# OpenVVC/OpenVVC

Measured on AMD Instinct MI355X. Metric: decoded frames/sec, full rcn back-end decode step (H2D of the recorded picture + MC incl. BDOF/DMVR/affine-PROF/GPM/CIIP + LMCS + inverse transform + ordered intra pass + deblocking + SAO + ALF/CC-ALF + D2H of refined MVs + wait + per-picture digest + publication to the device DPB), 4K 10-bit RA rec, higher is better.
Workload: dtype u16 samples / int16 coefficients / int32 accumulate

## Files before the change

openvvc_amd/csrc/kernels_mc.hip:

```cpp
#include "mc_common.hip.h"
#include <stdlib.h>

#ifndef OV_WPE_MC
#define OV_WPE_MC 8
#endif
#if OV_WPE_MC > 0
#define OV_OCC_MC __attribute__((amdgpu_waves_per_eu(OV_WPE_MC)))
#else
#define OV_OCC_MC
#endif

namespace {

__device__ __forceinline__ int mc_gpm(uint32_t aux, int x, int y, int p0, int p1)
{
    const int k = (int16_t)(aux & 0xffff), a = (int8_t)((aux >> 16) & 0xff), b = (int8_t)(aux >> 24);
    const int wgt = ov_clip3((k + __mul24(a, x) + __mul24(b, y)) >> 3, 0, 8);
    return ov_clip_bd((__mul24(p1, 8 - wgt) + __mul24(p0, wgt) + 64) >> 7);
}

struct Combine { int a0, a1, rnd, sh; };
__device__ __forceinline__ Combine mc_combine_of(const ovhip_mc_unit &u)
{
    Combine c;
    if (u.dir != 3)                 { c.a0 = u.dir == 1; c.a1 = u.dir != 1; c.rnd = 8; c.sh = 4; }
    else if (u.w0 == 4 && u.w1 == 4) { c.a0 = 1; c.a1 = 1; c.rnd = 16; c.sh = 5; }
    else                            { c.a0 = u.w0; c.a1 = u.w1; c.rnd = 64; c.sh = 7; }
    return c;
}
__device__ __forceinline__ int mc_combine(const Combine &c, int p0, int p1) { return ov_clip_bd((__mul24(p1, c.a1) + __mul24(p0, c.a0) + c.rnd) >> c.sh); }

__device__ __forceinline__ int ciip_blend(int inter, int intra, int wt) { return ov_clip_bd((__mul24(intra, wt) + __mul24(inter, 4 - wt) + 2) >> 2); }

#define HLS 26
template <int NOUT>
__device__ __forceinline__ void luma_finish(const ovhip_mc_unit &u, const ovhip_pic &dst, const int16_t *s_hl, const int tv[2][4],
                                            int lane, int log2w, const uint16_t *__restrict__ lmcs_fwd, const ovhip_pic &intra)
{
    const int w = 1 << log2w;
    const int x = lane & (w - 1), yg = lane >> log2w, y0 = yg * NOUT;
    if (y0 >= u.h) return;
    int P[2][NOUT];
#pragma unroll
    for (int l = 0; l < 2; ++l) {
#pragma unroll
        for (int o = 0; o < NOUT; ++o) P[l][o] = 0;
        if (u.dir & (1 << l)) v_outputs<8, NOUT>(s_hl + l * 16 * HLS + x * HLS, y0, tv[l], P[l]);
    }
    uint16_t *d = dst.y + ov_rowoff(u.y + y0, dst.stride_y) + u.x + x;
    int v[NOUT];
    if (u.flags & OVHIP_MC_GPM) {
#pragma unroll
        for (int j = 0; j < NOUT; ++j) v[j] = mc_gpm(u.aux, x, y0 + j, P[0][j], P[1][j]);
    } else {
        const Combine cmb = mc_combine_of(u);
#pragma unroll
        for (int j = 0; j < NOUT; ++j) v[j] = mc_combine(cmb, P[0][j], P[1][j]);
    }
    if ((u.flags & OVHIP_MC_LMCS) && lmcs_fwd) {
#pragma unroll
        for (int j = 0; j < NOUT; ++j) v[j] = lmcs_fwd[v[j]];
    }
    if (!(u.flags & OVHIP_MC_GPM) && u.aux) {
        const uint16_t *ip = intra.y + ov_rowoff(u.y + y0, intra.stride_y) + u.x + x;
#pragma unroll
        for (int j = 0; j < NOUT; ++j) v[j] = ciip_blend(v[j], ip[j * intra.stride_y], u.aux & 7);
    }
#pragma unroll
    for (int j = 0; j < NOUT; ++j) d[j * dst.stride_y] = (uint16_t)v[j];
}

template <int NOUT>
__device__ __forceinline__ void chroma_finish(const ovhip_mc_unit &u, const ovhip_pic &dst, const int16_t *s_hc, const int tv[2][2],
                                              int lane, int log2wc, int hc, const ovhip_pic &intra)
{
    const int wc = 1 << log2wc;
    const int per_plane = (wc * hc) / NOUT;
    const int plane = lane >= per_plane, ll = lane - plane * per_plane;
    if (lane >= 2 * per_plane) return;
    const int x = ll & (wc - 1), y0 = (ll >> log2wc) * NOUT;
    int P[2][NOUT];
#pragma unroll
    for (int l = 0; l < 2; ++l) {
#pragma unroll
        for (int o = 0; o < NOUT; ++o) P[l][o] = 0;
        if (u.dir & (1 << l)) v_outputs<4, NOUT>(s_hc + (plane * 2 + l) * 8 * CHT_STRIDE + x * CHT_STRIDE, y0, tv[l], P[l]);
    }
    uint16_t *d = (plane ? dst.cr : dst.cb) + ov_rowoff((u.y >> 1) + y0, dst.stride_c) + (u.x >> 1) + x;
    const bool ciip = !(u.flags & OVHIP_MC_GPM) && u.aux && !(u.aux & 0x100);
    const uint16_t *ip = ciip ? (plane ? intra.cr : intra.cb) + ov_rowoff((u.y >> 1) + y0, intra.stride_c) + (u.x >> 1) + x : nullptr;
    int v[NOUT];
    if (u.flags & OVHIP_MC_GPM) {
#pragma unroll
        for (int j = 0; j < NOUT; ++j) v[j] = mc_gpm(u.aux, 2 * x, 2 * (y0 + j), P[0][j], P[1][j]);
    } else {
        const Combine cmb = mc_combine_of(u);
#pragma unroll
        for (int j = 0; j < NOUT; ++j) v[j] = mc_combine(cmb, P[0][j], P[1][j]);
    }
    if (ciip) {
#pragma unroll
        for (int j = 0; j < NOUT; ++j) v[j] = ciip_blend(v[j], ip[j * intra.stride_c], u.aux & 7);
    }
#pragma unroll
    for (int j = 0; j < NOUT; ++j) d[j * dst.stride_c] = (uint16_t)v[j];
}

#ifdef OV_MC_PHASES
#define OV_MC_PHASE_UNITS 65536
__device__ unsigned int g_mc_phase[OV_MC_PHASE_UNITS * 8];
#define OV_PHASE(i) do { __builtin_amdgcn_s_waitcnt(0); const unsigned long long t_ = __builtin_readcyclecounter(); \
                         ph[i] = t_ - tprev; tprev = t_; } while (0)
#else
#define OV_PHASE(i) do { } while (0)
#endif

__global__ __launch_bounds__(64) OV_OCC_MC void k_mc2(ovhip_pic dst, RefTable refs, const ovhip_mc_unit *__restrict__ units,
                                             uint32_t n_units, const uint16_t *__restrict__ lmcs_fwd, int xcd, ovhip_pic intra)
{
    constexpr int HL_STRIDE = HLS;
    constexpr int R2 = 2 * 16 * HL_STRIDE > 4 * CHR_WIN ? 2 * 16 * HL_STRIDE : 4 * CHR_WIN;
    __shared__ __attribute__((aligned(16))) uint16_t s_all[2 * LUMA_WIN + R2 + 4 * 8 * CHT_STRIDE + 8];
    uint16_t *const s_wl = s_all;
    uint16_t *const s_wc = s_all + 2 * LUMA_WIN;
    int16_t  *const s_hl = reinterpret_cast<int16_t *>(s_all + 2 * LUMA_WIN);
    int16_t  *const s_hc = reinterpret_cast<int16_t *>(s_all + 2 * LUMA_WIN + R2);
    static_assert(sizeof(s_all) <= 5120, "k_mc2 LDS block must stay under the 32-workgroups-per-CU step");

    const int lane = threadIdx.x;
    {
    const uint32_t wg = blockIdx.x;
    if (wg >= n_units) return;
    const uint32_t bid = xcd ? ov_xcd_slot(wg, n_units) : wg;
#ifdef OV_MC_PHASES
    unsigned long long ph[8] = {}, tprev = __builtin_readcyclecounter();
#endif
    const ovhip_mc_unit u = units[bid];
    OV_PHASE(0);

    const bool do_l = !(u.flags & OVHIP_MC_NO_LUMA), do_c = !(u.flags & OVHIP_MC_NO_CHROMA);
    const int w = u.w, h = u.h, wc = w >> 1, hc = h >> 1;
    const int log2w = 31 - __clz(w), log2wc = log2w - 1;
    const int nl = u.dir == 3 ? 2 : 1, l0 = u.dir == 2 ? 1 : 0;

    const int ri0 = (u.dir & 1) ? u.ref0 : u.ref1, ri1 = (u.dir & 2) ? u.ref1 : u.ref0;
    const uint16_t *const ry[2]  = { refs.p[ri0].y,  refs.p[ri1].y };
    const uint16_t *const rcb[2] = { refs.p[ri0].cb, refs.p[ri1].cb };
    const uint16_t *const rcr[2] = { refs.p[ri0].cr, refs.p[ri1].cr };
    int lx[2], ly[2], cx[2], cy[2];
#pragma unroll
    for (int l = 0; l < 2; ++l) {
        const int mvx = l ? u.mv1x : u.mv0x, mvy = l ? u.mv1y : u.mv0y;
        lx[l] = u.x + (mvx >> 4) - 3;        ly[l] = u.y + (mvy >> 4) - 3;
        cx[l] = (u.x >> 1) + (mvx >> 5) - 1; cy[l] = (u.y >> 1) + (mvy >> 5) - 1;
    }
    const uint32_t (*const ltab)[4] = (u.flags & OVHIP_MC_FILT_4x4) ? g_taps.luma4 : g_taps.luma;
    const bool hpel = !(u.flags & OVHIP_MC_FILT_4x4) && (u.flags & OVHIP_MC_HPEL_FILT);
    const int hl_l = l0 + (nl == 2 ? lane >> 5 : 0);
    const int hc_q = lane >> (nl == 2 ? 4 : 5);
    const int hc_l = l0 + (nl == 2 ? (hc_q & 1) : 0);
    int fxl = (hl_l ? u.mv1x : u.mv0x) & 15;
    if (hpel && fxl == 8) fxl = 16;
    const int fxc = (hc_l ? u.mv1x : u.mv0x) & 31;
    const uint4 hl_tp = *reinterpret_cast<const uint4 *>(ltab[fxl]);
    const uint2 hc_tp = *reinterpret_cast<const uint2 *>(g_taps.chroma[fxc]);
    uint16_t *const lwin[2] = { s_wl, s_wl + LUMA_WIN };
    uint16_t *const cwin[4] = { s_wc, s_wc + CHR_WIN, s_wc + 2 * CHR_WIN, s_wc + 3 * CHR_WIN };
    int offl[2], offc1[2];
    stage_unit_windows(dst, ry, rcb, rcr, lx, ly, cx, cy, w, h, u.dir, do_l, do_c, lane, lwin, WIN_STRIDE, cwin, CWIN_STRIDE, offl, offc1);
    const int offc[2][2] = { { offc1[0], offc1[1] }, { offc1[0], offc1[1] } };
    __syncthreads();
    OV_PHASE(2);

    if (do_c) {
        const int log2seg = log2wc > 2 ? log2wc - 2 : 0;
        const int l2per = nl == 2 ? 4 : 5;
        const int qi = hc_q, tl = lane & ((1 << l2per) - 1);
        const int plane = nl == 2 ? qi >> 1 : qi, l = hc_l;
        const int tp[2] = { (int)hc_tp.x, (int)hc_tp.y };
        const int off = plane ? (l ? offc[1][1] : offc[1][0]) : (l ? offc[0][1] : offc[0][0]);
        const bool ident = fxc == 0;
        const uint16_t *src = s_wc + (plane * 2 + l) * CHR_WIN;
        int16_t *ht = s_hc + (plane * 2 + l) * 8 * CHT_STRIDE;
        const int x0 = (tl & ((1 << log2seg) - 1)) << 2, rstep = (1 << l2per) >> log2seg;
        for (int r = tl >> log2seg; r < hc + 3; r += rstep) h_task<4>(src + r * CWIN_STRIDE, off, x0, tp, ident, ht, CHT_STRIDE, r);
    }
    __syncthreads();
    if (do_l) {
        const int log2seg = log2w > 2 ? log2w - 2 : 0;
        const int l2per = nl == 2 ? 5 : 6;
        const int tl = lane & ((1 << l2per) - 1), l = hl_l;
        const int tp[4] = { (int)hl_tp.x, (int)hl_tp.y, (int)hl_tp.z, (int)hl_tp.w };
        const int off = l ? offl[1] : offl[0];
        const bool ident = fxl == 0;
        const uint16_t *src = s_wl + l * LUMA_WIN;
        int16_t *ht = s_hl + l * 16 * HL_STRIDE;
        const int x0 = (tl & ((1 << log2seg) - 1)) << 2, rstep = (1 << l2per) >> log2seg;
        for (int r = tl >> log2seg; r < h + 7; r += rstep) h_task<8>(src + r * WIN_STRIDE, off, x0, tp, ident, ht, HL_STRIDE, r);
    }
    __syncthreads();
    OV_PHASE(3);

    int tvl[2][4], tvc[2][2];
#pragma unroll
    for (int l = 0; l < 2; ++l) {
        const int mvy = l ? u.mv1y : u.mv0y;
        int fy = mvy & 15;
        if (hpel && fy == 8) fy = 16;
        load_taps<4>(ltab[fy], tvl[l]);
        load_taps<2>(g_taps.chroma[mvy & 31], tvc[l]);
    }
    if (do_l) {
        const int npix = w * h;
        if (npix >= 256)      luma_finish<4>(u, dst, s_hl, tvl, lane, log2w, lmcs_fwd, intra);
        else if (npix >= 128) luma_finish<2>(u, dst, s_hl, tvl, lane, log2w, lmcs_fwd, intra);
        else                  luma_finish<1>(u, dst, s_hl, tvl, lane, log2w, lmcs_fwd, intra);
    }
    if (do_c) {
        if (wc * hc >= 64) chroma_finish<2>(u, dst, s_hc, tvc, lane, log2wc, hc, intra);
        else               chroma_finish<1>(u, dst, s_hc, tvc, lane, log2wc, hc, intra);
    }
    __syncthreads();
#ifdef OV_MC_PHASES
    { const unsigned long long t_ = __builtin_readcyclecounter(); ph[4] = t_ - tprev; tprev = t_; }
    OV_PHASE(5);
    if (lane == 0 && bid < OV_MC_PHASE_UNITS) {
#pragma unroll
        for (int i = 0; i < 6; ++i) g_mc_phase[bid * 8 + i] = (unsigned int)ph[i];
        g_mc_phase[bid * 8 + 7] = 1;
    }
#endif
    }
}

__global__ __launch_bounds__(256) void k_ciip(ovhip_pic dst, ovhip_pic intra, const ovhip_ciip_unit *__restrict__ units, uint32_t n)
{
    for (uint32_t bid = blockIdx.x; bid < n; bid += gridDim.x) {
        const ovhip_ciip_unit u = units[bid];
#pragma unroll
        for (int plane = 0; plane < 3; ++plane) {
            const int c = plane != 0;
            if (c && u.chroma_inter) continue;
            const int lw = u.log2_w - c, w = 1 << lw, npix = w << (u.log2_h - c);
            int ds, is;
            uint16_t *d = ov_plane(dst, plane, ds) + (u.y >> c) * ds + (u.x >> c);
            const uint16_t *s = ov_plane(intra, plane, is) + (u.y >> c) * is + (u.x >> c);
            for (int t = threadIdx.x; t < npix; t += 256) {
                const int x = t & (w - 1), y = t >> lw;
                d[y * ds + x] = (uint16_t)ov_clip_bd((s[y * is + x] * u.wt + d[y * ds + x] * (4 - u.wt) + 2) >> 2);
            }
        }
    }
}

}

#ifdef OV_MC_PHASES
extern "C" int ovhip_debug_mc_phases(unsigned int *out )
{
    return hipMemcpyFromSymbol(out, HIP_SYMBOL(g_mc_phase), sizeof(unsigned int) * OV_MC_PHASE_UNITS * 8) == hipSuccess ? OVHIP_OK : OVHIP_ELAUNCH;
}
#endif

extern "C" int ovhip_ciip_launch(ovhip_ctx *ctx, const ovhip_pic *dst, const ovhip_pic *intra,
                                 const ovhip_ciip_unit *d_units, uint32_t n_units)
{
    if (!ctx || !dst || !intra) return OVHIP_EINVAL;
    OV_DEVICE(ctx);
    if (!n_units) return OVHIP_OK;
    if (!d_units) return ov_fail(ctx, OVHIP_EINVAL, "ovhip_ciip_launch: null units", hipSuccess);
    hipLaunchKernelGGL(k_ciip, dim3(n_units), dim3(256), 0, ctx->stream, *dst, *intra, d_units, n_units);
    OV_LAUNCH_CHECK(ctx, "k_ciip");
    return OVHIP_OK;
}

extern "C" int ovhip_mc_launch(ovhip_ctx *ctx, const ovhip_pic *dst, const ovhip_pic *refs, uint32_t n_refs,
                               const ovhip_mc_unit *d_units, uint32_t n_units, const uint16_t *d_lmcs_fwd_lut,
                               const ovhip_pic *intra)
{
    if (!ctx || !dst) return OVHIP_EINVAL;
    OV_DEVICE(ctx);
    if (!n_units) return OVHIP_OK;
    if (!refs || !n_refs || n_refs > MC_MAX_REFS || !d_units)
        return ov_fail(ctx, OVHIP_EINVAL, "ovhip_mc_launch: bad reference table / units", hipSuccess);
    RefTable t;
    memset(&t, 0, sizeof(t));
    for (uint32_t i = 0; i < n_refs; ++i) {
        if (refs[i].w != dst->w || refs[i].h != dst->h || refs[i].stride_y != dst->stride_y || refs[i].stride_c != dst->stride_c)
            return ov_fail(ctx, OVHIP_EUNSUP, "ovhip_mc_launch: reference picture geometry differs from dst (RPR)", hipSuccess);
        t.p[i] = refs[i];
    }
    for (uint32_t i = n_refs; i < MC_MAX_REFS; ++i) t.p[i] = refs[0];
    static int cfg_xcd = -1;
#ifdef OVHIP_TUNING
    if (cfg_xcd < 0) { const char *x = getenv("OVHIP_MC_XCD"); cfg_xcd = x ? atoi(x) : 1; }
#else
    cfg_xcd = 1;
#endif
    hipLaunchKernelGGL(k_mc2, dim3(n_units), dim3(64), 0, ctx->stream, *dst, t, d_units, n_units, d_lmcs_fwd_lut, cfg_xcd,
                       intra ? *intra : *dst);
    OV_LAUNCH_CHECK(ctx, "k_mc2");
    return OVHIP_OK;
}
```

Baseline: 3576.

## Specialise MC kernel per common block size and direction; skip integer-MV vertical filter

The per-unit MC body becomes a template over log2 width, log2 height and list count. The kernel dispatches the common 8/16 x 8/16 uni- and bi-pred cases to compile-time variants, with a generic fallback. L1-only units are canonicalised to L0, so the per-lane list offset disappears and the uni path loads only one tap set. A vertical filter with zero fractional MV now copies the centre tap instead of running the 8/4-tap FIR. The aim is fewer runtime branches and less ALU work in the hot MC path, at the cost of larger code size and possible register pressure. The trailing __syncthreads is also removed.

```diff
diff --git a/openvvc_amd/csrc/kernels_mc.hip b/openvvc_amd/csrc/kernels_mc.hip
--- a/openvvc_amd/csrc/kernels_mc.hip
+++ b/openvvc_amd/csrc/kernels_mc.hip
@@ -20,40 +20,53 @@
 }
 
 struct Combine { int a0, a1, rnd, sh; };
-__device__ __forceinline__ Combine mc_combine_of(const ovhip_mc_unit &u)
+__device__ __forceinline__ Combine mc_combine_of(int dir, int w0, int w1)
 {
     Combine c;
-    if (u.dir != 3)                 { c.a0 = u.dir == 1; c.a1 = u.dir != 1; c.rnd = 8; c.sh = 4; }
-    else if (u.w0 == 4 && u.w1 == 4) { c.a0 = 1; c.a1 = 1; c.rnd = 16; c.sh = 5; }
-    else                            { c.a0 = u.w0; c.a1 = u.w1; c.rnd = 64; c.sh = 7; }
+    if (dir != 3)               { c.a0 = dir == 1; c.a1 = dir != 1; c.rnd = 8; c.sh = 4; }
+    else if (w0 == 4 && w1 == 4) { c.a0 = 1; c.a1 = 1; c.rnd = 16; c.sh = 5; }
+    else                        { c.a0 = w0; c.a1 = w1; c.rnd = 64; c.sh = 7; }
     return c;
 }
 __device__ __forceinline__ int mc_combine(const Combine &c, int p0, int p1) { return ov_clip_bd((__mul24(p1, c.a1) + __mul24(p0, c.a0) + c.rnd) >> c.sh); }
 
 __device__ __forceinline__ int ciip_blend(int inter, int intra, int wt) { return ov_clip_bd((__mul24(intra, wt) + __mul24(inter, 4 - wt) + 2) >> 2); }
 
+template <int NT, int NOUT>
+__device__ __forceinline__ void v_list(const int16_t *col, int s0, const int tp[NT / 2], bool vid, int P[NOUT])
+{
+    if (vid) {
+#pragma unroll
+        for (int o = 0; o < NOUT; ++o) P[o] = col[s0 + NT / 2 - 1 + o];
+    } else {
+        v_outputs<NT, NOUT>(col, s0, tp, P);
+    }
+}
+
 #define HLS 26
-template <int NOUT>
-__device__ __forceinline__ void luma_finish(const ovhip_mc_unit &u, const ovhip_pic &dst, const int16_t *s_hl, const int tv[2][4],
-                                            int lane, int log2w, const uint16_t *__restrict__ lmcs_fwd, const ovhip_pic &intra)
+template <int NOUT, int NL>
+__device__ __forceinline__ void luma_finish(const ovhip_mc_unit &u, int dir, int h, const ovhip_pic &dst, const int16_t *s_hl,
+                                            const int tv[2][4], const bool vid[2], int lane, int log2w,
+                                            const uint16_t *__restrict__ lmcs_fwd, const ovhip_pic &intra)
 {
     const int w = 1 << log2w;
     const int x = lane & (w - 1), yg = lane >> log2w, y0 = yg * NOUT;
-    if (y0 >= u.h) return;
+    if (y0 >= h) return;
     int P[2][NOUT];
 #pragma unroll
     for (int l = 0; l < 2; ++l) {
 #pragma unroll
         for (int o = 0; o < NOUT; ++o) P[l][o] = 0;
-        if (u.dir & (1 << l)) v_outputs<8, NOUT>(s_hl + l * 16 * HLS + x * HLS, y0, tv[l], P[l]);
+        if ((dir >> l) & 1) v_list<8, NOUT>(s_hl + l * 16 * HLS + x * HLS, y0, tv[l], vid[l], P[l]);
     }
     uint16_t *d = dst.y + ov_rowoff(u.y + y0, dst.stride_y) + u.x + x;
+    const bool gpm = NL != 1 && (u.flags & OVHIP_MC_GPM);
     int v[NOUT];
-    if (u.flags & OVHIP_MC_GPM) {
+    if (gpm) {
 #pragma unroll
         for (int j = 0; j < NOUT; ++j) v[j] = mc_gpm(u.aux, x, y0 + j, P[0][j], P[1][j]);
     } else {
-        const Combine cmb = mc_combine_of(u);
+        const Combine cmb = mc_combine_of(dir, u.w0, u.w1);
 #pragma unroll
         for (int j = 0; j < NOUT; ++j) v[j] = mc_combine(cmb, P[0][j], P[1][j]);
     }
@@ -61,7 +74,7 @@
 #pragma unroll
         for (int j = 0; j < NOUT; ++j) v[j] = lmcs_fwd[v[j]];
     }
-    if (!(u.flags & OVHIP_MC_GPM) && u.aux) {
+    if (!gpm && u.aux) {
         const uint16_t *ip = intra.y + ov_rowoff(u.y + y0, intra.stride_y) + u.x + x;
 #pragma unroll
         for (int j = 0; j < NOUT; ++j) v[j] = ciip_blend(v[j], ip[j * intra.stride_y], u.aux & 7);
@@ -70,9 +83,9 @@
     for (int j = 0; j < NOUT; ++j) d[j * dst.stride_y] = (uint16_t)v[j];
 }
 
-template <int NOUT>
-__device__ __forceinline__ void chroma_finish(const ovhip_mc_unit &u, const ovhip_pic &dst, const int16_t *s_hc, const int tv[2][2],
-                                              int lane, int log2wc, int hc, const ovhip_pic &intra)
+template <int NOUT, int NL>
+__device__ __forceinline__ void chroma_finish(const ovhip_mc_unit &u, int dir, const ovhip_pic &dst, const int16_t *s_hc,
+                                              const int tv[2][2], const bool vid[2], int lane, int log2wc, int hc, const ovhip_pic &intra)
 {
     const int wc = 1 << log2wc;
     const int per_plane = (wc * hc) / NOUT;
@@ -84,17 +97,18 @@
     for (int l = 0; l < 2; ++l) {
 #pragma unroll
         for (int o = 0; o < NOUT; ++o) P[l][o] = 0;
-        if (u.dir & (1 << l)) v_outputs<4, NOUT>(s_hc + (plane * 2 + l) * 8 * CHT_STRIDE + x * CHT_STRIDE, y0, tv[l], P[l]);
+        if ((dir >> l) & 1) v_list<4, NOUT>(s_hc + (plane * 2 + l) * 8 * CHT_STRIDE + x * CHT_STRIDE, y0, tv[l], vid[l], P[l]);
     }
     uint16_t *d = (plane ? dst.cr : dst.cb) + ov_rowoff((u.y >> 1) + y0, dst.stride_c) + (u.x >> 1) + x;
-    const bool ciip = !(u.flags & OVHIP_MC_GPM) && u.aux && !(u.aux & 0x100);
+    const bool gpm = NL != 1 && (u.flags & OVHIP_MC_GPM);
+    const bool ciip = !gpm && u.aux && !(u.aux & 0x100);
     const uint16_t *ip = ciip ? (plane ? intra.cr : intra.cb) + ov_rowoff((u.y >> 1) + y0, intra.stride_c) + (u.x >> 1) + x : nullptr;
     int v[NOUT];
-    if (u.flags & OVHIP_MC_GPM) {
+    if (gpm) {
 #pragma unroll
         for (int j = 0; j < NOUT; ++j) v[j] = mc_gpm(u.aux, 2 * x, 2 * (y0 + j), P[0][j], P[1][j]);
     } else {
-        const Combine cmb = mc_combine_of(u);
+        const Combine cmb = mc_combine_of(dir, u.w0, u.w1);
 #pragma unroll
         for (int j = 0; j < NOUT; ++j) v[j] = mc_combine(cmb, P[0][j], P[1][j]);
     }
@@ -109,41 +123,37 @@
 #ifdef OV_MC_PHASES
 #define OV_MC_PHASE_UNITS 65536
 __device__ unsigned int g_mc_phase[OV_MC_PHASE_UNITS * 8];
+struct McPhases { unsigned long long ph[8], tprev; };
 #define OV_PHASE(i) do { __builtin_amdgcn_s_waitcnt(0); const unsigned long long t_ = __builtin_readcyclecounter(); \
-                         ph[i] = t_ - tprev; tprev = t_; } while (0)
+                         pc.ph[i] = t_ - pc.tprev; pc.tprev = t_; } while (0)
+#define OV_PHASE_ARG , McPhases &pc
+#define OV_PHASE_PASS , pc
 #else
 #define OV_PHASE(i) do { } while (0)
-#endif
-
-__global__ __launch_bounds__(64) OV_OCC_MC void k_mc2(ovhip_pic dst, RefTable refs, const ovhip_mc_unit *__restrict__ units,
-                                             uint32_t n_units, const uint16_t *__restrict__ lmcs_fwd, int xcd, ovhip_pic intra)
-{
-    constexpr int HL_STRIDE = HLS;
-    constexpr int R2 = 2 * 16 * HL_STRIDE > 4 * CHR_WIN ? 2 * 16 * HL_STRIDE : 4 * CHR_WIN;
-    __shared__ __attribute__((aligned(16))) uint16_t s_all[2 * LUMA_WIN + R2 + 4 * 8 * CHT_STRIDE + 8];
+#define OV_PHASE_ARG
+#define OV_PHASE_PASS
+#endif
+
+constexpr int MC2_R2 = 2 * 16 * HLS > 4 * CHR_WIN ? 2 * 16 * HLS : 4 * CHR_WIN;
+constexpr int MC2_LDS = 2 * LUMA_WIN + MC2_R2 + 4 * 8 * CHT_STRIDE + 8;
+static_assert(MC2_LDS * 2 <= 5120, "k_mc2 LDS block must stay under the 32-workgroups-per-CU step");
+
+template <int LW, int LH, int NL>
+__device__ __forceinline__ void mc2_unit(const ovhip_mc_unit &u, int lane, const ovhip_pic &dst, const RefTable &refs,
+                                         const uint16_t *__restrict__ lmcs_fwd, const ovhip_pic &intra, uint16_t *s_all OV_PHASE_ARG)
+{
     uint16_t *const s_wl = s_all;
     uint16_t *const s_wc = s_all + 2 * LUMA_WIN;
     int16_t  *const s_hl = reinterpret_cast<int16_t *>(s_all + 2 * LUMA_WIN);
-    int16_t  *const s_hc = reinterpret_cast<int16_t *>(s_all + 2 * LUMA_WIN + R2);
-    static_assert(sizeof(s_all) <= 5120, "k_mc2 LDS block must stay under the 32-workgroups-per-CU step");
-
-    const int lane = threadIdx.x;
-    {
-    const uint32_t wg = blockIdx.x;
-    if (wg >= n_units) return;
-    const uint32_t bid = xcd ? ov_xcd_slot(wg, n_units) : wg;
-#ifdef OV_MC_PHASES
-    unsigned long long ph[8] = {}, tprev = __builtin_readcyclecounter();
-#endif
-    const ovhip_mc_unit u = units[bid];
-    OV_PHASE(0);
+    int16_t  *const s_hc = reinterpret_cast<int16_t *>(s_all + 2 * LUMA_WIN + MC2_R2);
 
     const bool do_l = !(u.flags & OVHIP_MC_NO_LUMA), do_c = !(u.flags & OVHIP_MC_NO_CHROMA);
-    const int w = u.w, h = u.h, wc = w >> 1, hc = h >> 1;
-    const int log2w = 31 - __clz(w), log2wc = log2w - 1;
-    const int nl = u.dir == 3 ? 2 : 1, l0 = u.dir == 2 ? 1 : 0;
-
-    const int ri0 = (u.dir & 1) ? u.ref0 : u.ref1, ri1 = (u.dir & 2) ? u.ref1 : u.ref0;
+    const int log2w = LW ? LW : 31 - __clz(u.w), log2wc = log2w - 1;
+    const int w = 1 << log2w, h = LH ? 1 << LH : u.h, wc = w >> 1, hc = h >> 1;
+    const int dir = NL ? (NL == 2 ? 3 : 1) : u.dir;
+    const int nl = dir == 3 ? 2 : 1;
+
+    const int ri0 = (dir & 1) ? u.ref0 : u.ref1, ri1 = (dir & 2) ? u.ref1 : u.ref0;
     const uint16_t *const ry[2]  = { refs.p[ri0].y,  refs.p[ri1].y };
     const uint16_t *const rcb[2] = { refs.p[ri0].cb, refs.p[ri1].cb };
     const uint16_t *const rcr[2] = { refs.p[ri0].cr, refs.p[ri1].cr };
@@ -156,9 +166,9 @@
     }
     const uint32_t (*const ltab)[4] = (u.flags & OVHIP_MC_FILT_4x4) ? g_taps.luma4 : g_taps.luma;
     const bool hpel = !(u.flags & OVHIP_MC_FILT_4x4) && (u.flags & OVHIP_MC_HPEL_FILT);
-    const int hl_l = l0 + (nl == 2 ? lane >> 5 : 0);
+    const int hl_l = nl == 2 ? lane >> 5 : 0;
     const int hc_q = lane >> (nl == 2 ? 4 : 5);
-    const int hc_l = l0 + (nl == 2 ? (hc_q & 1) : 0);
+    const int hc_l = nl == 2 ? (hc_q & 1) : 0;
     int fxl = (hl_l ? u.mv1x : u.mv0x) & 15;
     if (hpel && fxl == 8) fxl = 16;
     const int fxc = (hc_l ? u.mv1x : u.mv0x) & 31;
@@ -166,9 +176,8 @@
     const uint2 hc_tp = *reinterpret_cast<const uint2 *>(g_taps.chroma[fxc]);
     uint16_t *const lwin[2] = { s_wl, s_wl + LUMA_WIN };
     uint16_t *const cwin[4] = { s_wc, s_wc + CHR_WIN, s_wc + 2 * CHR_WIN, s_wc + 3 * CHR_WIN };
-    int offl[2], offc1[2];
-    stage_unit_windows(dst, ry, rcb, rcr, lx, ly, cx, cy, w, h, u.dir, do_l, do_c, lane, lwin, WIN_STRIDE, cwin, CWIN_STRIDE, offl, offc1);
-    const int offc[2][2] = { { offc1[0], offc1[1] }, { offc1[0], offc1[1] } };
+    int offl[2], offc[2];
+    stage_unit_windows(dst, ry, rcb, rcr, lx, ly, cx, cy, w, h, dir, do_l, do_c, lane, lwin, WIN_STRIDE, cwin, CWIN_STRIDE, offl, offc);
     __syncthreads();
     OV_PHASE(2);
 
@@ -178,7 +187,7 @@
         const int qi = hc_q, tl = lane & ((1 << l2per) - 1);
         const int plane = nl == 2 ? qi >> 1 : qi, l = hc_l;
         const int tp[2] = { (int)hc_tp.x, (int)hc_tp.y };
-        const int off = plane ? (l ? offc[1][1] : offc[1][0]) : (l ? offc[0][1] : offc[0][0]);
+        const int off = l ? offc[1] : offc[0];
         const bool ident = fxc == 0;
         const uint16_t *src = s_wc + (plane * 2 + l) * CHR_WIN;
         int16_t *ht = s_hc + (plane * 2 + l) * 8 * CHT_STRIDE;
@@ -194,43 +203,76 @@
         const int off = l ? offl[1] : offl[0];
         const bool ident = fxl == 0;
         const uint16_t *src = s_wl + l * LUMA_WIN;
-        int16_t *ht = s_hl + l * 16 * HL_STRIDE;
+        int16_t *ht = s_hl + l * 16 * HLS;
         const int x0 = (tl & ((1 << log2seg) - 1)) << 2, rstep = (1 << l2per) >> log2seg;
-        for (int r = tl >> log2seg; r < h + 7; r += rstep) h_task<8>(src + r * WIN_STRIDE, off, x0, tp, ident, ht, HL_STRIDE, r);
+        for (int r = tl >> log2seg; r < h + 7; r += rstep) h_task<8>(src + r * WIN_STRIDE, off, x0, tp, ident, ht, HLS, r);
     }
     __syncthreads();
     OV_PHASE(3);
 
     int tvl[2][4], tvc[2][2];
+    bool vidl[2], vidc[2];
 #pragma unroll
     for (int l = 0; l < 2; ++l) {
         const int mvy = l ? u.mv1y : u.mv0y;
         int fy = mvy & 15;
         if (hpel && fy == 8) fy = 16;
+        vidl[l] = fy == 0; vidc[l] = (mvy & 31) == 0;
+        if (NL == 1 && l) continue;
         load_taps<4>(ltab[fy], tvl[l]);
         load_taps<2>(g_taps.chroma[mvy & 31], tvc[l]);
     }
     if (do_l) {
         const int npix = w * h;
-        if (npix >= 256)      luma_finish<4>(u, dst, s_hl, tvl, lane, log2w, lmcs_fwd, intra);
-        else if (npix >= 128) luma_finish<2>(u, dst, s_hl, tvl, lane, log2w, lmcs_fwd, intra);
-        else                  luma_finish<1>(u, dst, s_hl, tvl, lane, log2w, lmcs_fwd, intra);
+        if (npix >= 256)      luma_finish<4, NL>(u, dir, h, dst, s_hl, tvl, vidl, lane, log2w, lmcs_fwd, intra);
+        else if (npix >= 128) luma_finish<2, NL>(u, dir, h, dst, s_hl, tvl, vidl, lane, log2w, lmcs_fwd, intra);
+        else                  luma_finish<1, NL>(u, dir, h, dst, s_hl, tvl, vidl, lane, log2w, lmcs_fwd, intra);
     }
     if (do_c) {
-        if (wc * hc >= 64) chroma_finish<2>(u, dst, s_hc, tvc, lane, log2wc, hc, intra);
-        else               chroma_finish<1>(u, dst, s_hc, tvc, lane, log2wc, hc, intra);
-    }
-    __syncthreads();
+        if (wc * hc >= 64) chroma_finish<2, NL>(u, dir, dst, s_hc, tvc, vidc, lane, log2wc, hc, intra);
+        else               chroma_finish<1, NL>(u, dir, dst, s_hc, tvc, vidc, lane, log2wc, hc, intra);
+    }
+}
+
+__global__ __launch_bounds__(64) OV_OCC_MC void k_mc2(ovhip_pic dst, RefTable refs, const ovhip_mc_unit *__restrict__ units,
+                                             uint32_t n_units, const uint16_t *__restrict__ lmcs_fwd, int xcd, ovhip_pic intra)
+{
+    __shared__ __attribute__((aligned(16))) uint16_t s_all[MC2_LDS];
+
+    const int lane = threadIdx.x;
+    const uint32_t wg = blockIdx.x;
+    if (wg >= n_units) return;
+    const uint32_t bid = xcd ? ov_xcd_slot(wg, n_units) : wg;
 #ifdef OV_MC_PHASES
-    { const unsigned long long t_ = __builtin_readcyclecounter(); ph[4] = t_ - tprev; tprev = t_; }
+    McPhases pc = {};
+    pc.tprev = __builtin_readcyclecounter();
+#endif
+    ovhip_mc_unit u = units[bid];
+    OV_PHASE(0);
+    if (u.dir == 2) { u.dir = 1; u.ref0 = u.ref1; u.mv0x = u.mv1x; u.mv0y = u.mv1y; }
+
+    const int nl = u.dir == 3 ? 2 : (u.dir == 1 && !(u.flags & OVHIP_MC_GPM)) ? 1 : 0;
+    const bool sized = ((u.w == 8) | (u.w == 16)) & ((u.h == 8) | (u.h == 16));
+    switch (nl && sized ? (u.w >> 4) * 4 + (u.h >> 4) * 2 + nl - 1 : 8) {
+    case 0:  mc2_unit<3, 3, 1>(u, lane, dst, refs, lmcs_fwd, intra, s_all OV_PHASE_PASS); break;
+    case 1:  mc2_unit<3, 3, 2>(u, lane, dst, refs, lmcs_fwd, intra, s_all OV_PHASE_PASS); break;
+    case 2:  mc2_unit<3, 4, 1>(u, lane, dst, refs, lmcs_fwd, intra, s_all OV_PHASE_PASS); break;
+    case 3:  mc2_unit<3, 4, 2>(u, lane, dst, refs, lmcs_fwd, intra, s_all OV_PHASE_PASS); break;
+    case 4:  mc2_unit<4, 3, 1>(u, lane, dst, refs, lmcs_fwd, intra, s_all OV_PHASE_PASS); break;
+    case 5:  mc2_unit<4, 3, 2>(u, lane, dst, refs, lmcs_fwd, intra, s_all OV_PHASE_PASS); break;
+    case 6:  mc2_unit<4, 4, 1>(u, lane, dst, refs, lmcs_fwd, intra, s_all OV_PHASE_PASS); break;
+    case 7:  mc2_unit<4, 4, 2>(u, lane, dst, refs, lmcs_fwd, intra, s_all OV_PHASE_PASS); break;
+    default: mc2_unit<0, 0, 0>(u, lane, dst, refs, lmcs_fwd, intra, s_all OV_PHASE_PASS); break;
+    }
+#ifdef OV_MC_PHASES
+    { const unsigned long long t_ = __builtin_readcyclecounter(); pc.ph[4] = t_ - pc.tprev; pc.tprev = t_; }
     OV_PHASE(5);
     if (lane == 0 && bid < OV_MC_PHASE_UNITS) {
 #pragma unroll
-        for (int i = 0; i < 6; ++i) g_mc_phase[bid * 8 + i] = (unsigned int)ph[i];
+        for (int i = 0; i < 6; ++i) g_mc_phase[bid * 8 + i] = (unsigned int)pc.ph[i];
         g_mc_phase[bid * 8 + 7] = 1;
     }
 #endif
-    }
 }
 
 __global__ __launch_bounds__(256) void k_ciip(ovhip_pic dst, ovhip_pic intra, const ovhip_ciip_unit *__restrict__ units, uint32_t n)
```

Result: no change. 3535, median of 2 (-1.1%).
